# twosigma/Cook

Measured on AMD Instinct MI355X. Metric: match-cycles/sec at 1M pending x 50k offers, higher is better.
Workload: dtype f64

## Files before the change

### cook_amd/csrc/classfit_asm.hpp

```cpp
#pragma once
#if CF_SLOTS_N == 12
#define CF_O_CTRL "13728"
#define CF_O_CTRL4 "13732"
#define CF_O_ARR "15280"
#define CF_O_CLS32 "9504"
#define CF_SLOT_SHIFT "9"
#define CF_SLOT_N "12"
#elif CF_SLOTS_N == 24
#define CF_O_CTRL "16800"
#define CF_O_CTRL4 "16804"
#define CF_O_ARR "18352"
#define CF_O_CLS32 "12576"
#define CF_SLOT_SHIFT "10"
#define CF_SLOT_N "24"
#else
#error "CF_SLOTS_N: 12 or 24"
#endif
#ifndef CF_ASM_WAIT_READS
#define CF_ASM_WAIT_READS "30"
#endif
#define CF_ASM_MAX_STEP(ctrl) "v_max_f32_dpp v113, v113, v113 " ctrl "\n\ts_nop 1\n\t"
#define CF_ASM_DECIDER_STEP                                                                                                             \
  "v_readlane_b32 s60, v80, s44\n\t"                                                                                                    \
  "v_readlane_b32 s61, v81, s44\n\t"                                                                                                    \
  "v_readlane_b32 s62, v82, s44\n\t"                                                                                                    \
  "s_mov_b32 s41, 1\n\t"                                                                                                                \
  "s_and_b32 s63, s62, 0xffff00ff\n\t"                                                                                                   \
  "s_cmp_lg_u32 s63, 0\n\t"                                                                                                             \
  "s_cbranch_scc1 9f\n\t"                                                                                                               \
                                                                                           \
  "v_mov_b32_e32 v88, s47\n\t"                                                                                                          \
  "v_mov_b32_e32 v89, s51\n\t"                                                                                                          \
  "v_add_u32_e32 v100, s46, v83\n\t"                                                                                                    \
  "s_mov_b64 exec, 1\n\t"                                                                                                               \
  "ds_write_b32 v89, v88 offset:" CF_O_CTRL4 "\n\t"                                                                                              \
  "s_mov_b64 exec, -1\n\t"                                                                                                              \
  "s_mov_b32 s82, " CF_ASM_WAIT_READS "\n\t"              \
  "1:\n\t"                                                                                                                              \
  "ds_read_b32 v92, v100\n\t"                                                                                                           \
  "ds_read_b64 v[94:95], v100 offset:8\n\t"                                                                                             \
  "ds_read_b128 v[96:99], v100 offset:16\n\t"                                                                                           \
  "ds_read_b32 v93, v100\n\t"                                                                                                           \
  "v_lshlrev_b32_e32 v114, 3, v65\n\t"  \
  "v_add_u32_e32 v114, s56, v114\n\t"                                                                                                   \
  "ds_read_b64 v[114:115], v114\n\t"                                                                                                    \
                                        \
  "v_subrev_u32_e32 v101, s60, v71\n\t"                                                                                                 \
  "v_subrev_u32_e32 v102, s61, v72\n\t"                                                                                                 \
  "v_cvt_f64_u32_e32 v[104:105], v101\n\t"                                                                                              \
  "v_cvt_f64_u32_e32 v[106:107], v102\n\t"                                                                                              \
  "v_mul_f64 v[104:105], v[104:105], v[66:67]\n\t"                                                                                      \
  "v_mul_f64 v[106:107], v[106:107], v[68:69]\n\t"                                                                                      \
  "v_add_f64 v[104:105], v[104:105], v[106:107]\n\t"                                                                                    \
  "v_add_f64 v[104:105], -v[104:105], 1.0\n\t"                                                                                          \
  "v_cmp_le_u32_e64 s[64:65], s60, v71\n\t"                                                                                             \
  "v_cmp_le_u32_e64 s[66:67], s61, v72\n\t"                                                                                             \
  "v_cmp_ne_u32_e64 s[68:69], 0, v64\n\t"                                                                                               \
  "s_and_b64 s[64:65], s[64:65], s[66:67]\n\t"                                                                                          \
  "s_and_b64 s[64:65], s[64:65], s[68:69]\n\t"                                                                                          \
  "s_waitcnt lgkmcnt(0)\n\t"                                                                                                            \
        \
  "s_bfe_u32 s63, s62, 0x4000c\n\t"                                                                                                     \
  "s_cmp_eq_u32 s63, 0\n\t"                                                                                                             \
  "s_cbranch_scc1 3f\n\t"                                                                                                               \
  "v_readlane_b32 s66, v85, s44\n\t"                                                                                                    \
  "v_readlane_b32 s67, v86, s44\n\t"                                                                                                    \
  "s_cmp_lt_u32 s63, 1\n\t"                                                                                                           \
  "s_cbranch_scc1 3f\n\t"                                                                                                               \
  "s_bfe_u32 s72, s66, 0x100000\n\t"                                                                      \
  "s_lshr_b32 s73, s72, 8\n\t"                                                                                                          \
  "s_lshl_b32 s73, s73, 3\n\t"                                                                                                          \
  "s_and_b32 s72, s72, 0xff\n\t"                                                                                                        \
  "v_lshrrev_b64 v[108:109], s73, v[114:115]\n\t"                                                                                       \
  "v_and_b32_e32 v108, 0xff, v108\n\t"                                                                                                  \
  "v_cmp_eq_u32_e64 s[74:75], s72, v108\n\t"                                                                                            \
  "s_and_b64 s[64:65], s[64:65], s[74:75]\n\t"                                                                                          \
  "s_cmp_lt_u32 s63, 2\n\t"                                                                                                           \
  "s_cbranch_scc1 3f\n\t"                                                                                                               \
  "s_bfe_u32 s72, s66, 0x100010\n\t"                                                                      \
  "s_lshr_b32 s73, s72, 8\n\t"                                                                                                          \
  "s_lshl_b32 s73, s73, 3\n\t"                                                                                                          \
  "s_and_b32 s72, s72, 0xff\n\t"                                                                                                        \
  "v_lshrrev_b64 v[108:109], s73, v[114:115]\n\t"                                                                                       \
  "v_and_b32_e32 v108, 0xff, v108\n\t"                                                                                                  \
  "v_cmp_eq_u32_e64 s[74:75], s72, v108\n\t"                                                                                            \
  "s_and_b64 s[64:65], s[64:65], s[74:75]\n\t"                                                                                          \
  "s_cmp_lt_u32 s63, 3\n\t"                                                                                                           \
  "s_cbranch_scc1 3f\n\t"                                                                                                               \
  "s_bfe_u32 s72, s67, 0x100000\n\t"                                                                      \
  "s_lshr_b32 s73, s72, 8\n\t"                                                                                                          \
  "s_lshl_b32 s73, s73, 3\n\t"                                                                                                          \
  "s_and_b32 s72, s72, 0xff\n\t"                                                                                                        \
  "v_lshrrev_b64 v[108:109], s73, v[114:115]\n\t"                                                                                       \
// ... 23 lines not shown
  "v_cmp_ne_u32_e64 s[78:79], v109, v75\n\t"                                                                                            \
  "v_cmp_gt_i32_e64 s[80:81], 0, v95\n\t"                                                                                               \
  "s_and_b64 s[74:75], s[74:75], s[76:77]\n\t"                                                                                          \
  "s_and_b64 s[74:75], s[74:75], s[78:79]\n\t"                                                                                          \
  "s_or_b64 s[74:75], s[74:75], s[80:81]\n\t"                                                                                           \
  "s_and_b64 s[72:73], s[70:71], s[72:73]\n\t"                                          \
  "s_and_b64 s[70:71], s[72:73], s[74:75]\n\t"                                                                                            \
  "s_andn2_b64 s[76:77], s[52:53], s[70:71]\n\t"                                                                     \
  "s_cmp_eq_u64 s[76:77], 0\n\t"                                                                                                          \
  "s_cbranch_scc1 2f\n\t"                                                                                                                 \
   \
   \
  "s_and_b64 s[78:79], s[76:77], s[72:73]\n\t"                                                                                            \
  "s_cmp_eq_u64 s[78:79], 0\n\t"                                                                                                          \
  "s_cbranch_scc1 4f\n\t"                                                                                                                 \
  "v_and_b32_e32 v109, 0x3fff, v95\n\t"                                                                                                   \
  "s_and_b64 s[72:73], s[64:65], s[54:55]\n\t"                                                   \
  "10:\n\t"                                                                                                                               \
  "s_ff1_i32_b64 s83, s[78:79]\n\t"                                                                                                       \
  "v_readlane_b32 s63, v109, s83\n\t"                                                                                                     \
  "s_bitset0_b64 s[78:79], s83\n\t"                                                                                                       \
  "v_cmp_eq_u32_e64 vcc, s63, v65\n\t"                                                                                                    \
  "s_and_b64 vcc, vcc, s[72:73]\n\t"                                                                                                      \
  "s_cmp_eq_u64 vcc, 0\n\t"                                                                                                               \
  "s_cbranch_scc1 11f\n\t"                                                                                                                \
  "s_bitset1_b64 s[80:81], s83\n\t"                                                                                                       \
  "s_bitset0_b64 s[76:77], s83\n\t"                                                                                                       \
  "11:\n\t"                                                                                                                               \
  "s_cmp_lg_u64 s[78:79], 0\n\t"                                                                                                          \
  "s_cbranch_scc1 10b\n\t"                                                                                                                \
  "s_cmp_eq_u64 s[76:77], 0\n\t"                                                                                                          \
  "s_cbranch_scc1 2f\n\t"                                                                                                                 \
  "4:\n\t"                                                                                                                                \
  "s_sub_u32 s82, s82, 1\n\t"      \
  "s_cmp_eq_u32 s82, 0\n\t"                                                                                                             \
  "s_cbranch_scc1 9f\n\t"                                                                                                               \
  "s_sleep 1\n\t"                                                                                                                       \
  "s_branch 1b\n\t"                                                                                                                     \
  "2:\n\t"                                                                                                                              \
  "s_andn2_b64 s[74:75], s[52:53], s[80:81]\n\t"                                                                        \
  "s_or_b64 s[64:65], s[64:65], s[74:75]\n\t"                                                          \
  "v_cndmask_b32_e64 v110, v98, v104, s[54:55]\n\t"                                                                                     \
  "v_cndmask_b32_e64 v111, v99, v105, s[54:55]\n\t"                                                                                     \
  "v_cndmask_b32_e64 v110, 0, v110, s[64:65]\n\t"                                                                                       \
  "v_cndmask_b32_e64 v111, 0, v111, s[64:65]\n\t"                                                                                       \
  "v_cvt_f32_f64_e32 v112, v[110:111]\n\t"                                                                                              \
  "s_nop 0\n\t"                                                                                                                         \
  "v_mov_b32_e32 v113, v112\n\t"                                                                                                        \
  "s_nop 1\n\t"                                                                                                                         \
  CF_ASM_MAX_STEP("quad_perm:[1,0,3,2] row_mask:0xf bank_mask:0xf")                                                                     \
  CF_ASM_MAX_STEP("quad_perm:[2,3,0,1] row_mask:0xf bank_mask:0xf")                                                                     \
  CF_ASM_MAX_STEP("row_half_mirror row_mask:0xf bank_mask:0xf")                                                                         \
  CF_ASM_MAX_STEP("row_mirror row_mask:0xf bank_mask:0xf")                                                                              \
  CF_ASM_MAX_STEP("row_bcast:15 row_mask:0xa bank_mask:0xf")                                                                            \
  CF_ASM_MAX_STEP("row_bcast:31 row_mask:0xc bank_mask:0xf")                                                                            \
  "v_readlane_b32 s63, v113, 63\n\t"                                                                                                    \
  "s_mov_b32 s41, 0\n\t"                                                                                                                \
  "s_cmp_eq_u32 s63, 0\n\t"                                                                                                             \
  "s_cbranch_scc1 9f\n\t"                                                                                          \
  "s_mov_b32 s41, 1\n\t"                                                                                                                \
  "v_cmp_eq_f32_e64 s[78:79], s63, v112\n\t"                                                                                            \
  "v_add_f32_e32 v108, 0x35000000, v112\n\t"                                                                               \
  "v_cmp_le_f32_e64 s[76:77], s63, v108\n\t"                                                                                            \
  "v_and_b32_e32 v109, 0x40000000, v95\n\t"                                                                                             \
  "v_cmp_ne_u32_e64 s[70:71], 0, v109\n\t"                                                                                              \
  "s_and_b64 s[76:77], s[76:77], s[64:65]\n\t"                                      \
  "s_bcnt1_i32_b64 s62, s[76:77]\n\t"                                                                                                   \
  "s_cmp_gt_u32 s62, 1\n\t"                                                                                                             \
  "s_cbranch_scc1 9f\n\t"                                                                                                               \
  "s_and_b64 s[70:71], s[70:71], s[76:77]\n\t"                                                                                          \
  "s_and_b64 s[70:71], s[70:71], s[74:75]\n\t"                       \
  "s_cmp_lg_u64 s[70:71], 0\n\t"                                                                                                        \
  "s_cbranch_scc1 9f\n\t"                                                                                                               \
  "s_ff1_i32_b64 s82, s[78:79]\n\t"                                                                                                     \
  "s_cmp_lt_u32 s82, 58\n\t"                                                                                                            \
  "s_cbranch_scc0 5f\n\t"                                                                                                               \
                                                                                                         \
  "v_readlane_b32 s64, v71, s82\n\t"                                                                                                    \
  "v_readlane_b32 s65, v72, s82\n\t"                                                                                                    \
  "v_readlane_b32 s66, v65, s82\n\t"                                                                                                    \
  "s_sub_u32 s67, s64, s60\n\t"                                                                                                         \
  "s_sub_u32 s70, s65, s61\n\t"                                                                                                         \
  "v_cmp_eq_u32_e64 vcc, s82, v84\n\t"                                                                                                  \
  "v_mov_b32_e32 v88, s67\n\t"                                                                                                          \
  "v_mov_b32_e32 v89, s70\n\t"                                                                                                          \
  "s_cmp_lt_u32 s67, s49\n\t"                                                                                                           \
  "s_cselect_b32 s71, 1, 0\n\t"                                                                                                         \
  "s_cmp_lt_u32 s70, s50\n\t"                                                                                                           \
  "s_cselect_b32 s62, 1, 0\n\t"                                                                                                         \
  "s_or_b32 s71, s71, s62\n\t"                                                                                                          \
  "v_cndmask_b32_e32 v71, v71, v88, vcc\n\t"                                                                                            \
  "v_cndmask_b32_e32 v72, v72, v89, vcc\n\t"                                                                                            \
  "s_cmp_lg_u32 s71, 0\n\t"                                                                                                             \
  "s_cselect_b64 s[62:63], vcc, 0\n\t"                             \
  "s_mov_b32 s72, s44\n\t"                                                                                                              \
  "s_mov_b32 s73, 0\n\t"                                                                                                                \
  "v_cndmask_b32_e64 v64, v64, 0, s[62:63]\n\t"                                                                                         \
  "s_branch 7f\n\t"                                                                                                                     \
        \
  "5:\n\t"                                                                                                                              \
  "v_readlane_b32 s64, v96, s82\n\t"                                                                                                    \
  "v_readlane_b32 s65, v97, s82\n\t"                                                                                                    \
  "v_readlane_b32 s76, v95, s82\n\t"                                                                                                    \
  "v_readlane_b32 s77, v94, s82\n\t"                                                                                                    \
  "v_readlane_b32 s78, v73, s82\n\t"                                                                                                    \
  "s_sub_u32 s67, s64, s60\n\t"                                                                                                         \
// ... 33 lines not shown
  "s_nop 0\n\t"                                                                                                                         \
  "v_cndmask_b32_e32 v75, v75, v74, vcc\n\t"                                                                                            \
  "v_cndmask_b32_e32 v74, v74, v101, vcc\n\t"                                                                                           \
  "v_cndmask_b32_e32 v73, v73, v100, vcc\n\t"                                                                                           \
  "s_lshl_b32 s62, s80, 8\n\t"                                                                                                          \
  "s_lshl_b32 s63, s81, 12\n\t"                                                                                                         \
  "s_or_b32 s72, s44, s62\n\t"                                                                                                          \
  "s_or_b32 s72, s72, s63\n\t"                                                                                                          \
  "s_cmp_lg_u32 s71, 0\n\t"                                                                                                             \
  "s_cbranch_scc1 7f\n\t"                                                                              \
  "s_mul_i32 s62, s79, 56\n\t"                                                                                                          \
  "s_add_u32 s62, s62, s51\n\t"                                                                                                         \
  "v_mov_b32_e32 v90, s62\n\t"                                                                                                          \
  "ds_read_b128 v[116:119], v90 offset:" CF_O_CLS32 "\n\t"                                                                                        \
  "s_andn2_b64 s[62:63], s[54:55], s[68:69]\n\t"                                                                                        \
  "s_ff1_i32_b64 s83, s[62:63]\n\t"                                                                                                     \
  "v_cmp_eq_u32_e64 vcc, s83, v84\n\t"                                                                                                  \
  "v_mov_b32_e32 v88, s66\n\t"                                                                                                          \
  "v_mov_b32_e32 v89, s79\n\t"                                                                                                          \
  "v_mov_b32_e32 v91, s67\n\t"                                                                                                          \
  "v_mov_b32_e32 v101, s70\n\t"                                                                                                         \
  "v_cndmask_b32_e64 v64, v64, 1, vcc\n\t"                                                                                              \
  "v_cndmask_b32_e32 v65, v65, v88, vcc\n\t"                                                                                            \
  "v_cndmask_b32_e32 v70, v70, v89, vcc\n\t"                                                                                            \
  "v_cndmask_b32_e32 v71, v71, v91, vcc\n\t"                                                                                            \
  "v_cndmask_b32_e32 v72, v72, v101, vcc\n\t"                                                                                           \
  "s_waitcnt lgkmcnt(0)\n\t"                                                                                                            \
  "v_cndmask_b32_e32 v66, v66, v116, vcc\n\t"                                                                                           \
  "v_cndmask_b32_e32 v67, v67, v117, vcc\n\t"                                                                                           \
  "v_cndmask_b32_e32 v68, v68, v118, vcc\n\t"                                                                                           \
  "v_cndmask_b32_e32 v69, v69, v119, vcc\n\t"                                                                                           \
   \
  "7:\n\t"                                                                                                                              \
  "v_cmp_eq_u32_e64 vcc, s44, v84\n\t"                                                                                                  \
  "v_mov_b32_e32 v88, s66\n\t"                                                                                                          \
  "v_cmp_lt_u32_e64 s[62:63], s67, v80\n\t"                                                                                             \
  "v_cmp_lt_u32_e64 s[76:77], s70, v81\n\t"                                                                                             \
  "v_cndmask_b32_e32 v76, v76, v88, vcc\n\t"                                                                                            \
  "s_or_b64 s[62:63], s[62:63], s[76:77]\n\t"                                                                                           \
  "s_lshl_b64 s[76:77], -2, s44\n\t"                                                                                                    \
  "s_and_b64 s[62:63], s[62:63], s[76:77]\n\t"                                                                                          \
  "s_or_b64 s[38:39], s[38:39], s[62:63]\n\t"                                                                                           \
  "s_min_u32 s37, s37, s67\n\t"                                                                                                         \
  "s_min_u32 s40, s40, s70\n\t"                                                                                                         \
  "s_add_u32 s36, s36, 1\n\t"                                                                                                           \
  "v_mov_b32_e32 v88, s72\n\t"                                                                                                          \
  "v_mov_b32_e32 v89, s73\n\t"                                                                                                          \
  "v_mov_b32_e32 v90, s64\n\t"                                                                                                          \
  "v_mov_b32_e32 v91, s65\n\t"                                                                                                          \
  "v_mov_b32_e32 v100, s48\n\t"                                                                                                         \
  "s_mov_b64 exec, 1\n\t"                                                                                                               \
  "ds_write_b128 v100, v[88:91]\n\t"                                                                                                    \
  "s_mov_b64 exec, -1\n\t"                                                                                                              \
  "s_mov_b32 s41, 2\n\t"                                                                                                                \
  "9:\n\t"

#define CF_ASM_CLASS_STEP                                                                                                               \
  "v_mov_b32_e32 v80, s44\n\t"                                                                                                          \
  "s_lshl_b32 s60, s45, 2\n\t"                                                                                                          \
  "s_add_u32 s60, s60, s44\n\t"                                                                                                         \
  "v_mov_b32_e32 v81, s60\n\t"                                                                                                          \
  "ds_read_b64 v[82:83], v80 offset:" CF_O_CTRL "\n\t"                                                                     \
  "ds_read_b32 v84, v81 offset:" CF_O_CTRL4 "\n\t"                                                                   \
  "s_mov_b32 s41, 3\n\t"                                                                                                                \
  "s_waitcnt lgkmcnt(0)\n\t"                                                                                                            \
  "v_readfirstlane_b32 s61, v82\n\t"                                                                                                    \
  "v_readfirstlane_b32 s42, v83\n\t"                                                                                                    \
  "v_readfirstlane_b32 s43, v84\n\t"                                                                                                    \
  "s_cmp_lg_u32 s61, 0\n\t"                                                                                                             \
  "s_cbranch_scc1 9f\n\t"                                                                                                               \
  "s_cmp_lg_u32 s43, s40\n\t"                                                                                                           \
  "s_cbranch_scc1 9f\n\t"                                                                                                               \
  "s_mov_b32 s41, 2\n\t"                                                                                                                \
                                                                                                 \
  "1:\n\t"                                                                                                                              \
  "s_cmp_eq_u64 s[36:37], 0\n\t"                                                                                                        \
  "s_cbranch_scc1 9f\n\t"                                                                                                               \
  "s_cmp_eq_u32 s39, s56\n\t"                                                                                                           \
  "s_cbranch_scc1 2f\n\t"                                                                                                               \
  "s_add_u32 s62, s36, -1\n\t"                                                                                                          \
  "s_addc_u32 s63, s37, -1\n\t"                                                                                                         \
  "s_and_b64 s[36:37], s[36:37], s[62:63]\n\t"                                                                                          \
  "s_add_u32 s38, s38, 1\n\t"                                                                                                           \
  "s_add_u32 s39, s39, 1\n\t"                                                                                                           \
  "s_cmp_eq_u32 s39, s57\n\t"                                                                                                           \
  "s_cselect_b32 s39, 0, s39\n\t"                                                                                                       \
  "s_branch 1b\n\t"                                                                                                                     \
  "2:\n\t"                                                                                                                                \
// ... 123 lines not shown
```

### cook_amd/csrc/classfit_walk.hpp

```cpp
#pragma once
#if defined(CF_PROF) && !defined(CF_STATS)
#define CF_STATS 1
#endif
#ifdef CF_STATS
#define CF_STAT(x) x
#define CF_TICKS() cook_ticks()
#else
#define CF_STAT(x) ((void)0)
#define CF_TICKS() 0ull
#endif
#ifdef CF_PROF
#define CF_PROF_T(x) const unsigned long long x = __builtin_readcyclecounter()
#define CF_PROF_ADD(i, d) prof[i] += (unsigned long long)(d)
#else
#define CF_PROF_T(x) ((void)0)
#define CF_PROF_ADD(i, d) ((void)0)
#endif

#ifndef CF_AHEAD
#define CF_AHEAD 10
#endif
constexpr unsigned CF_BOARD = CF_AHEAD;
#ifndef CF_SLOTS_N
#define CF_SLOTS_N 12
// ... 285 lines not shown
  v.id = (unsigned)wave_read_lane((int)p.w0, (int)wl), v.pos = (unsigned)wave_read_lane((int)p.pos, (int)wl), v.fc = (unsigned)wave_read_lane((int)p.fc, (int)wl),
  v.fm = (unsigned)wave_read_lane((int)p.fm, (int)wl), v.cls = (unsigned)wave_read_lane((int)p.cls, (int)wl), v.aux = (unsigned)wave_read_lane((int)p.aux, (int)wl);
  return v;
}
static __device__ __forceinline__ unsigned cf_poll(const uint32_t* p) { return (unsigned)wave_read_lane((int)ld_wg(p), 0); }
static __device__ __forceinline__ unsigned long long cf_below(unsigned s) { return (1ull << s) - 1ull; }

enum : unsigned { CFE_K = 0, CFE_M, CFE_NP, CFE_NCLS, CFE_NKIND, CFE_CMIN, CFE_MMIN, CFE_KC, CFE_KM, CFE_MINFC, CFE_MINFM, CFE_N = 12 };
constexpr float CF_BAND32 = 1.0f / 2097152.0f;

struct CfFixed {
  CfEnt board[CF_SLOTS * 8u];
  CfLog log[64];
  CfJob ring[2u * 64u];
  CfPost post2[8];
  CfClass cls[CF_MAXCLS];
  uint32_t pw[8u * CF_LV], aw[8u * CF_LV], gk[CF_MAXKIND * CF_LV], ovt[CF_LV];
  uint32_t ctrl[8];
  uint32_t ovl[192], ckept[3u * CF_MAXCLS], misc[CFX_N];
  uint32_t env_t[CF_LV], envw[CFE_N];
};
static_assert(sizeof(CfFixed) % 16 == 0, "the arrays behind it are 16-byte aligned");
#if COOK_HAS_ASM_WALK
#define CF_ASM_EPOCH_LIVE "57"
#include "classfit_asm.hpp"
static_assert(CF_EPOCH_AT == 58 && CF_OVL == 58, "classfit_asm.hpp: the overlay's size");
static_assert(offsetof(CfFixed, ctrl) == 13728 + (CF_SLOTS - 12) * 256 && offsetof(CfFixed, cls) == 9472 + (CF_SLOTS - 12) * 256 && sizeof(CfFixed) == 15280 + (CF_SLOTS - 12) * 256 && sizeof(CfClass) == 56 && offsetof(CfClass, hTc) == 32 &&
                  offsetof(CfClass, hTm) == 40 && offsetof(CfEnt, pos) == 8 && offsetof(CfEnt, cid) == 12 && offsetof(CfEnt, fc) == 16 && offsetof(CfEnt, fa) == 24 && sizeof(CfEnt) == 32 &&
                  sizeof(CfLog) == 32 && offsetof(CfLog, ofc) == 8,
              "classfit_asm.hpp: offsets of the LDS records");
typedef unsigned cf_u32x16 __attribute__((ext_vector_type(16)));
typedef unsigned cf_u32x8 __attribute__((ext_vector_type(8)));
typedef unsigned cf_u32x4 __attribute__((ext_vector_type(4)));
#endif

template <int ROLE>
static __device__ __forceinline__ void cf_walk_role(const CfLds& S, const MatchState& st, const CfBuf& b, const unsigned lw, const unsigned rep, const unsigned nrep,
                                                    const unsigned long long t_start) {
  constexpr bool is_decider = ROLE == 0, is_class_wave = ROLE == 1, is_books = ROLE == 2;
  const unsigned tid = threadIdx.x, lane = lane_id();
  CfCtl* ctl = b.ctl;
  const unsigned K = wave_uniform_u32(S.envw[CFE_K]), cmin = wave_uniform_u32(S.envw[CFE_CMIN]), mmin = wave_uniform_u32(S.envw[CFE_MMIN]);
  const uint32_t* t = S.t;
#define n_cls wave_uniform_u32(S.envw[CFE_NCLS])
#define n_kind wave_uniform_u32(S.envw[CFE_NKIND])
#define NP wave_uniform_u32(S.envw[CFE_NP])
  CfChunkLane c;
  unsigned nch_wave = 0;
  cf_setup_chunks(S.cls, n_cls, is_class_wave ? lw : 0xFFu, lane, c, nch_wave);
  c.lv = CfLv8{0u, 0u, 0u, 0u, 0u, 0u, 0u, 0u}, c.la = c.lv;
  unsigned my_kinds = 0;
  {
    const unsigned forw = is_class_wave ? lw : (is_decider && lane >= CF_OVL ? lane - CF_OVL + 1u : 0xFFu);
    for (unsigned ci = 0; ci < n_cls; ++ci)
      if (S.cls[ci].wave == forw && S.cls[ci].kind < 32u) my_kinds |= 1u << S.cls[ci].kind;
  }
  const unsigned wk = is_class_wave ? wave_uniform_u32(my_kinds) : 0u;
  unsigned one_cls = 0xFFFFFFFFu, u_off = 0, u_n = 0;
  double u_hTc = 0.0, u_hTm = 0.0;
  auto class_setup = [&] {
    unsigned cnt = 0, ci0 = 0;
    for (unsigned ci = 0; ci < n_cls; ++ci)
      if (S.cls[ci].wave == lw) ++cnt, ci0 = ci;
    one_cls = cnt == 1u ? ci0 : 0xFFFFFFFFu;
    const CfClass* cl = &S.cls[ci0];
    u_off = cl->off, u_n = cl->n, u_hTc = cl->hTc, u_hTm = cl->hTm;
  };
  if (is_class_wave) {
    class_setup();
    for (unsigned ch = 0; ch < nch_wave; ++ch) cf_tighten(S, lane, ch, c);
    if (rep == 0u && lw != 0u) cf_wave_tables(S, lw, lane, c, wk, n_kind);
  }
  CfOvLane o;
  o.valid = 0u, o.id = 0u, o.cls = 0u, o.fc = 0u, o.fm = 0u, o.hTc = 0.0, o.hTm = 0.0;
  unsigned nrm = 0, rm1 = 0xFFFFFFFFu, rm2 = 0xFFFFFFFFu;
  unsigned minfc_all = wave_uniform_u32(S.envw[CFE_MINFC]), minfm_all = wave_uniform_u32(S.envw[CFE_MINFM]);
  unsigned matched = 0, head = 0;
  unsigned jc = 0, jm = 0, jmeta = 0, jgrp = 0, jeq0 = 0, jeq1 = 0, jnov0 = 0, jnov1 = 0;
  int res = -1;
  unsigned long long b1m = 0ull;
  unsigned seen = 0, gen = 0;
  unsigned tight_applied = 0;
  bool bk_room0 = false, nx_room0 = false, nx_walk = false;
  unsigned st_scans = 0, st_exact = 0, st_open = 0, st_ovwin = 0, st_gpu = 0, st_epochs = 0, st_tight = 0, st_walked = 0, st_dead = 0, st_opendead = 0, st_spins = 0, st_flips = 0,
           st_rewinds = 0;
  unsigned long long tk_epoch = 0, tk_books = 0, tk_walk = 0, tk_phase1 = 0;
#ifdef CF_PROF
  unsigned long long prof[8] = {0, 0, 0, 0, 0, 0, 0, 0};
#endif
  auto job_of = [&](unsigned s) -> CfJobU {
    CfJobU J;
    J.c = (unsigned)wave_read_lane((int)jc, (int)s), J.m = (unsigned)wave_read_lane((int)jm, (int)s);
    const unsigned meta = (unsigned)wave_read_lane((int)jmeta, (int)s);
    J.kind = meta & 255u, J.L = (meta >> 8) & 15u, J.n_eq = (meta >> 12) & 15u, J.n_nov = (meta >> 16) & 15u, J.grouped = (meta >> 20) & 1u;
    J.grp = 0u, J.eq0 = J.eq1 = 0u, J.nov0 = J.nov1 = 0xFFFFFFFFu;
    if (meta >> 12) {
      J.grp = (unsigned)wave_read_lane((int)jgrp, (int)s), J.eq0 = (unsigned)wave_read_lane((int)jeq0, (int)s), J.eq1 = (unsigned)wave_read_lane((int)jeq1, (int)s),
      J.nov0 = (unsigned)wave_read_lane((int)jnov0, (int)s), J.nov1 = (unsigned)wave_read_lane((int)jnov1, (int)s);
    }
    return J;
  };
  auto tables_room_any = [&](unsigned L, unsigned m) -> bool {
    bool r = S.ovt[L] > m;
    for (unsigned x = 1; x <= (unsigned)CF_CW; ++x) r = r || S.aw[x * CF_LV + L] > m;
    return r;
  };
  auto tables_walk = [&](unsigned kind, unsigned L, unsigned m) -> bool {
    bool r = false;
    if (kind == 0u) {
      r = S.ovt[L] > m;
      for (unsigned x = 1; x <= (unsigned)CF_CW; ++x) r = r || S.pw[x * CF_LV + L] > m;
    } else if (kind < (unsigned)CF_MAXKIND) {
      r = S.gk[kind * CF_LV + L] > m;
    }
    return r;
  };
  CfJob nxt;
  nxt.c = nxt.m = nxt.meta = nxt.grp = nxt.eq[0] = nxt.eq[1] = nxt.nov[0] = nxt.nov[1] = 0u;
  auto books_next = [&](unsigned nbase) {
    const unsigned nn = nbase < K ? cf_min(64u, K - nbase) : 0u;
    const unsigned nslot = (nbase >> 6) & 1u;
// ... 38 lines not shown
    unsigned cur_ord = 0;
    unsigned ph = 0;
    bool batch_done = nw == 0u;
    const unsigned long long tw0 = CF_TICKS();
    CF_PROF_T(cw0);
    while (!batch_done) {
      unsigned md = 0;
      if (is_decider) {
#if COOK_HAS_ASM_WALK
        cf_u32x16 ST = {0u, 0u, 0u, 0u, 0u, 0u, 0u, 0u, 0u, 0u, 0u, 0u, 0u, 0u, 0u, 0u};
        cf_u32x8 JB = {jc, jm, jmeta, clw * 32u, lane, jeq0, jeq1, 0u};
        const unsigned long long rel0 = cook_ballot(!isov & ((my_kinds & 1u) != 0u)), ovm = cf_below(CF_OVL);
        const cf_u32x8 MK = {wave_uniform_u32((unsigned)rel0), wave_uniform_u32((unsigned)(rel0 >> 32)), wave_uniform_u32((unsigned)ovm), wave_uniform_u32((unsigned)(ovm >> 32)),
                             wave_uniform_u32(cook_lds_off(S.attr8)), 0u, 0u, 0u};
        const unsigned a_board = wave_uniform_u32(cook_lds_off(S.board)), a_log = wave_uniform_u32(cook_lds_off(S.log));
        auto st_pack = [&] {
          const unsigned long long hc = (unsigned long long)__double_as_longlong(o.hTc), hm = (unsigned long long)__double_as_longlong(o.hTm);
          ST[0] = o.valid, ST[1] = o.id, ST[2] = (unsigned)hc, ST[3] = (unsigned)(hc >> 32), ST[4] = (unsigned)hm, ST[5] = (unsigned)(hm >> 32), ST[6] = o.cls, ST[7] = o.fc, ST[8] = o.fm,
          ST[9] = nrm, ST[10] = rm1, ST[11] = rm2, ST[12] = (unsigned)res;
        };
        auto st_unpack = [&] {
          o.valid = ST[0], o.id = ST[1], o.hTc = __longlong_as_double((long long)((unsigned long long)ST[3] << 32 | ST[2])),
          o.hTm = __longlong_as_double((long long)((unsigned long long)ST[5] << 32 | ST[4])), o.cls = ST[6], o.fc = ST[7], o.fm = ST[8], nrm = ST[9], rm1 = ST[10], rm2 = ST[11],
          res = (int)ST[12];
        };
#endif
        while (md == 0u) {
          todo = wave_uniform_u64(todo), cur_ord = wave_uniform_u32(cur_ord), logn = wave_uniform_u32(logn), matched = wave_uniform_u32(matched), gen = wave_uniform_u32(gen);
          minfc_all = wave_uniform_u32(minfc_all), minfm_all = wave_uniform_u32(minfm_all), b1m = wave_uniform_u64(b1m);
#if COOK_HAS_ASM_WALK
          {
            st_pack();
            CF_PROF_T(f0);
            while (todo != 0ull) {
              const unsigned fs = (unsigned)__ffsll(todo) - 1u;
#define CF_U(x) wave_uniform_u32((unsigned)(x))
              cf_u32x8 SC = {CF_U(matched), CF_U(minfc_all), CF_U(b1m), CF_U(b1m >> 32), CF_U(minfm_all), 1u, 0u, 0u};
              const cf_u32x8 AR = {CF_U(fs), CF_U((base + fs) << 12 | (gen & 15u) << 8), CF_U(a_board + cf_slot(cur_ord) * 8u * (unsigned)sizeof(CfEnt)), CF_U(fs | cur_ord << 8),
                                   CF_U(a_log + logn * (unsigned)sizeof(CfLog)), CF_U(cmin), CF_U(mmin), a_board};
#undef CF_U
              asm volatile(CF_ASM_DECIDER_STEP
                           : "+{v[64:79]}"(ST), "+{s[36:43]}"(SC)
                           : "{v[80:87]}"(JB), "{s[44:51]}"(AR), "{s[52:59]}"(MK)
                           : "v88", "v89", "v90", "v91", "v92", "v93", "v94", "v95", "v96", "v97", "v98", "v99", "v100", "v101", "v102", "v103", "v104", "v105", "v106", "v107", "v108",
                             "v109", "v110", "v111", "v112", "v113", "v114", "v115", "v116", "v117", "v118", "v119", "s60", "s61", "s62", "s63", "s64", "s65", "s66", "s67", "s68", "s69",
                             "s70", "s71", "s72", "s73", "s74", "s75", "s76", "s77", "s78", "s79", "s80", "s81", "s82", "s83", "vcc", "scc", "memory");
#ifdef CF_DELAY_D
              __builtin_amdgcn_s_sleep(6);
#endif
              const unsigned status = wave_uniform_u32(SC[5]);
              if (status == 1u) break;
              matched = wave_uniform_u32(SC[0]), minfc_all = wave_uniform_u32(SC[1]), minfm_all = wave_uniform_u32(SC[4]);
              b1m = wave_uniform_u64((unsigned long long)SC[3] << 32 | SC[2]);
              logn += status >> 1;
              todo &= todo - 1ull, ++cur_ord;
              CF_PROF_ADD(4, 1);
            }
            CF_PROF_T(f1);
            CF_PROF_ADD(5, f1 - f0);
            WAIT_LDS();
            st_unpack();
          }
#endif
          if (todo == 0ull) {
            md = CFM_BATCH_END;
            st_lane0_b32(&S.ctrl[0], md);
            break;
          }
          CF_PROF_T(p0);
          const unsigned s = (unsigned)__ffsll(todo) - 1u;
          const unsigned ord = cur_ord;
          st_lane0_b32(&S.ctrl[1], s | ord << 8);
          const unsigned Jc = (unsigned)wave_read_lane((int)jc, (int)s), Jm = (unsigned)wave_read_lane((int)jm, (int)s), meta = (unsigned)wave_read_lane((int)jmeta, (int)s);
          const unsigned kind = meta & 255u;
          const unsigned want = (base + s) << 12 | (gen & 15u) << 8;
          const CfEnt* e = &S.board[cf_slot(ord) * 8u + clw];
          const bool relevant = !isov && kind < 32u && ((my_kinds >> (kind & 31u)) & 1u);
          unsigned cpos, ccid, cfc, cfm;
          double cfa;
          bool acc;
          bool ok_ov = isov & (o.valid != 0u) & (kind == 0u) & (o.fc >= Jc) & (o.fm >= Jm);
          if (meta >> 12) {
            const CfJobU J = job_of(s);
            ok_ov = ok_ov & cf_cons_ok(S, J, o.id, ok_ov);
          }
          for (;;) {
            const unsigned t1 = ld_wg(&e->tag);
            COMPILER_FENCE();
            cpos = e->pos, ccid = e->cid, cfc = e->fc, cfm = e->fm, cfa = e->fa;
// ... 550 lines not shown
        if (unm) {
          fail = (((bb >> lane) & 1ull) ? 1u : 0u) | (room ? 2u : 0u);
          if (fail == 0u) fail = 8u;
        }
        st.fail_code[base + lane] = fail;
      }
      books_next(base + 64u);
      bk_room0 = nx_room0;
      if (base + 128u + lane < K) nxt = b.jobs[base + 128u + lane];
      tk_books += CF_TICKS() - tb0;
    }
    EMU_SITE("classfit: batch end");
    __syncthreads();
  }
  if (is_decider) {
    if (lane == 0) {
      st.summary[0] = matched;
      st.summary[1] = (matched == 0u || head) ? 1u : 0u;
      st.summary[2] = st_epochs;
      const unsigned long long t_end = cook_ticks();
      uint32_t* sx = ctl->stats;
      sx[CFS_MATCHED] = matched, sx[CFS_OV_WIN] = st_ovwin, sx[CFS_OPEN] = st_open, sx[CFS_OPEN_DEAD] = st_opendead, sx[CFS_GPU_PLACE] = st_gpu, sx[CFS_EPOCHS] = st_epochs,
      sx[CFS_EXACT] = st_exact, sx[CFS_WALKED] = st_walked, sx[CFS_DEAD_DROP] = st_dead, sx[CFS_BATCHES] = (K + 63u) / 64u, sx[CFS_PRESETTLED] = K - st_walked;
      sx[CFS_TICKS_TOTAL] = (uint32_t)(t_end - t_start), sx[CFS_TICKS_PROLOGUE] = (uint32_t)(t_loop - t_start), sx[CFS_TICKS_EPOCH] = (uint32_t)tk_epoch;
      sx[CFS_TICKS_WALK] = (uint32_t)tk_walk, sx[CFS_TICKS_PHASE1] = (uint32_t)tk_phase1;
      sx[CFS_HWID_DECIDER] = cook_hw_id();
    }
    const unsigned sp = wave_max_u32(!isov ? st_spins : 0u);
    if (lane == 0) ctl->stats[CFS_SPINS] = sp;
  }
  if (is_class_wave && lane == 0) atomicAdd(&ctl->stats[CFS_SCANS], st_scans), atomicAdd(&ctl->stats[CFS_TIGHTEN], st_tight), atomicAdd(&ctl->stats[CFS_REWINDS], st_rewinds);
  if (is_books && lane == 0) ctl->stats[CFS_TICKS_PRECHECK] = (uint32_t)tk_books, ctl->stats[CFS_FLIPS] = st_flips, ctl->stats[CFS_HWID_BOOKS] = cook_hw_id();
#ifdef CF_PROF
  if (lane == 0 && (is_decider || (is_class_wave && lw >= 1u && lw <= 2u && rep == 0u)))
    for (int i = 0; i < 8; ++i) ctl->stats[24 + 8 * (is_decider ? 0u : lw) + i] = (uint32_t)(prof[i] >> 4);
#endif
#undef n_cls
#undef n_kind
#undef NP
}

static __device__ __forceinline__ void cf_walk_pool(char* lds, const MatchIn* __restrict__ inp, const MatchState& st, const CfBuf& b) {
  const unsigned tid = threadIdx.x, lane = lane_id(), w = wave_id();
  CfCtl* ctl = b.ctl;
  const unsigned K = inp->K, M = ctl->M, G = inp->G;
  const unsigned NP = (M + 63u) & ~63u;
  const unsigned long long t_start = cook_ticks();
  const bool any_eq = ctl->any_eq != 0u, any_group = ctl->any_group != 0u;
  __shared__ unsigned s_total, s_wsum[CF_WAVES];
  constexpr unsigned GPT = CF_MAXG / CF_THREADS;
  unsigned gsz[GPT];
  unsigned gsum = 0;
#pragma unroll
  for (unsigned x = 0; x < GPT; ++x) {
    const unsigned g = tid * GPT + x;
    unsigned sz = 0;
    if (any_group && g < G && b.gcount[g] != 0u) sz = (inp->g_run_off ? inp->g_run_off[g + 1] - inp->g_run_off[g] : 0u) + b.gcount[g];
    gsz[x] = sz, gsum += sz;
  }
  unsigned incl = gsum;
  for (unsigned d = 1; d < 64u; d <<= 1) {
    const unsigned y = shfl_up_t<unsigned>(incl, d);
    if (lane >= d) incl += y;
  }
  if (lane == 63u) s_wsum[w] = incl;
  __syncthreads();
  unsigned wbase = 0;
  for (unsigned x = 0; x < w; ++x) wbase += s_wsum[x];
// ... 115 lines not shown
```

### cook_amd/csrc/engine.hip

```cpp
#include <hip/hip_runtime.h>
#include <sys/mman.h>
#include <ucontext.h>

#include <algorithm>
#include <atomic>
#include <cmath>
#include <cstdlib>
#include <chrono>
#include <cstring>
#include <limits>
#include <functional>
#include <map>
#include <string>
#include <tuple>
#include <vector>

#include "../../include/cookmatch.h"
#include "common.hpp"
#include "multi.hpp"
#include "considerable_kernels.hpp"
#include "match_kernels.hpp"
#include "match_v2.hpp"
#include "classfit.hpp"
#include "offers_kernels.hpp"
// ... 1297 lines not shown
  return true;
}
void cf_run(cook_engine* lead, cook_engine* const* es, unsigned n, hipStream_t stream) {
  cook_engine* e = lead;
  for (unsigned i0 = 0; i0 < n; i0 += (unsigned)CF_PACK) {
    const unsigned c = std::min<unsigned>(CF_PACK, n - i0);
    CfPack pk{};
    for (unsigned x = 0; x < (unsigned)CF_PACK; ++x) pk.c[x] = es[i0 + (x < c ? x : 0u)]->deferred_cf;
    KLS("cf_walk", stream, cf_walk, c, CF_THREADS, pk);
  }
  for (unsigned i = 0; i < n; ++i) {
    const CfPoolCtx& c = es[i]->deferred_cf;
    const unsigned G = es[i]->last_in.G;
    if (G) KLS("cf_group_chains", stream, cf_group_chains, div_up(G, 256), 256, c.b, c.st, G);
  }
  constexpr size_t SLOT = 16 + 48 * 4;
  if (!lead->h_cf) COOK_HIP(hipHostMalloc((void**)&lead->h_cf, 64 * SLOT, hipHostMallocDefault));
  if (n > 64) lead->fail(COOK_E_INVALID, "cook_cycle_match_multi: at most 64 pools per call");
  for (unsigned i = 0; i < n; ++i) {
    char* slot = lead->h_cf + i * SLOT;
    COOK_HIP(hipMemcpyAsync(slot, es[i]->deferred_cf.st.summary, 16, hipMemcpyDeviceToHost, stream));
    COOK_HIP(hipMemcpyAsync(slot + 16, es[i]->deferred_cf.b.ctl->stats, 48 * 4, hipMemcpyDeviceToHost, stream));
  }
  COOK_HIP(hipStreamSynchronize(stream));
  for (unsigned i = 0; i < n; ++i) {
    cook_engine* x = es[i];
    const unsigned* sum = (const unsigned*)(lead->h_cf + i * SLOT);
    if (sum[3] == 0xDEADu) lead->fail(COOK_E_STATE, "cf_walk: the pool's tables do not fit the workgroup's LDS (the host's check let it through)");
    std::memcpy(x->cf_stats, lead->h_cf + i * SLOT + 16, 48 * 4);
#ifdef CF_PROF
    {
      const uint32_t* q = x->cf_stats;
      std::fprintf(stderr, "CFPROF (x16 shader cycles) decider: slow steps %u (candidates %u evaluation %u commit %u) plain steps %u in %u walk-total %u | class wave 1: poll %u answer %u answers %u idle %u idles %u | class wave 2: poll %u answer %u answers %u idle %u idles %u | walk ticks(100MHz) %u\n", q[27], q[24], q[25], q[26], q[28], q[29], q[31], q[32], q[33], q[35], q[36], q[37], q[40], q[41], q[43], q[44], q[45], q[CFS_TICKS_WALK]);
    }
#endif
    WinCtl c{};
    c.matched = sum[0], c.head_matched = sum[1], c.rounds = sum[2], c.head = x->last_in.K, c.visited_sum = x->cf_stats[CFS_WALKED];
    c.t_seq = x->cf_stats[CFS_TICKS_TOTAL], c.t_setup = x->cf_stats[CFS_TICKS_PROLOGUE];
    x->last_ctl = c;
    x->last_form = 3;
    x->has_deferred_cf = false;
    x->has_deferred = false;
    x->match_done = true;
  }
}

void match_run_device(cook_engine* e, unsigned K, const uint32_t* j_index, bool defer = false) {
  MatchIn in = e->min;
  in.K = K;
  in.j_index = j_index;
  in.good_enough = e->params.good_enough_fitness;
  in.host_lifetime_mins = e->params.host_lifetime_mins;
  const unsigned M = in.M, G = in.G;
  e->last_in = in;
  e->last_in_valid = true;
  MatchState st;
  st.ac = e->m_ac.ensure(M);
  st.am = e->m_am.ensure(M);
  st.acount = e->m_acount.ensure(M);
  st.group_last = e->m_group_last.ensure(G);
  st.job_prev = e->m_job_prev.ensure(K);
  st.job_to_offer = e->m_j2o.ensure(K);
  st.fail_code = e->m_fail.ensure(K);
  st.summary = e->m_summary.ensure(4);
  st.alive = e->m_alive.ensure((M + 63u) / 64u + 1u);
  st.jmin = (const double*)e->m_jmin.ensure(4);
// ... 1295 lines not shown
```

Before: 21.15.

## Run decider loop inside inline asm and prefetch next slot's row during commit

The decider's per-step loop moves from C++ into the assembly block, so one asm call walks every bit in the todo mask and the per-step register marshalling and exit checks go away. During each step's commit path it issues the LDS reads for the next slot's row early, so the next step can skip those reads and only post its head word. The loads are waited on with partial lgkmcnt counts instead of a full drain. This adds complexity and relies on careful lgkmcnt accounting, and opt-in profiling hooks for the individual phases are added as well.

```diff
diff --git a/cook_amd/csrc/classfit_asm.hpp b/cook_amd/csrc/classfit_asm.hpp
--- a/cook_amd/csrc/classfit_asm.hpp
+++ b/cook_amd/csrc/classfit_asm.hpp
@@ -19,8 +19,57 @@
 #ifndef CF_ASM_WAIT_READS
 #define CF_ASM_WAIT_READS "30"
 #endif
+#define CF_ASM_READ_ROW(addr)                                                                                                           \
+  "ds_read_b32 v92, " addr "\n\t"                                                                                                       \
+  "ds_read_b64 v[94:95], " addr " offset:8\n\t"                                                                                         \
+  "ds_read_b128 v[96:99], " addr " offset:16\n\t"                                                                                       \
+  "ds_read_b32 v93, " addr "\n\t"                                                                                                       \
+  "v_lshlrev_b32_e32 v114, 3, v65\n\t"                                                                                                  \
+  "v_add_u32_e32 v114, s56, v114\n\t"                                                                                                   \
+  "ds_read_b64 v[114:115], v114\n\t"
+#define CF_ASM_HEAD_WORD "s_mov_b64 exec, 1\n\tds_write_b32 v89, v88 offset:" CF_O_CTRL4 "\n\ts_mov_b64 exec, -1\n\t"
+#ifdef CF_PROF_PHASES
+#define CF_ASM_WAIT_COLD "s_waitcnt lgkmcnt(0)\n\t"
+#define CF_ASM_WAIT_EARLY "s_waitcnt lgkmcnt(0)\n\t"
+#else
+#define CF_ASM_WAIT_COLD "s_waitcnt lgkmcnt(1)\n\t"
+#define CF_ASM_WAIT_EARLY "s_waitcnt lgkmcnt(2)\n\t"
+#endif
 #define CF_ASM_MAX_STEP(ctrl) "v_max_f32_dpp v113, v113, v113 " ctrl "\n\ts_nop 1\n\t"
-#define CF_ASM_DECIDER_STEP                                                                                                             \
+#ifdef CF_DELAY_D
+#define CF_ASM_DELAY_D "s_sleep 6\n\t"
+#else
+#define CF_ASM_DELAY_D ""
+#endif
+#ifdef CF_PROF_PHASES
+#define CF_ASM_PS(acc) "s_memtime s[84:85]\n\ts_waitcnt lgkmcnt(0)\n\ts_sub_u32 s86, s84, s87\n\ts_add_u32 " acc ", " acc ", s86\n\ts_mov_b32 s87, s84\n\t"
+#define CF_ASM_PS_ENTRY "s_memtime s[84:85]\n\ts_waitcnt lgkmcnt(0)\n\ts_mov_b32 s87, s84\n\t"
+#define CF_ASM_PS_TOP "s_memtime s[84:85]\n\t"
+#define CF_ASM_PS_READ "s_sub_u32 s86, s84, s87\n\ts_add_u32 s92, s92, s86\n\ts_mov_b32 s87, s84\n\t" CF_ASM_PS("s88")
+#define CF_ASM_PS_REREAD "s_add_u32 s93, s93, 1\n\t"
+#else
+#define CF_ASM_PS(acc) ""
+#define CF_ASM_PS_ENTRY ""
+#define CF_ASM_PS_TOP ""
+#define CF_ASM_PS_READ ""
+#define CF_ASM_PS_REREAD ""
+#endif
+#define CF_ASM_DECIDER_RUN                                                                                                              \
+  CF_ASM_PS_ENTRY                                                                                                                       \
+                     \
+  "0:\n\t"                                                                                                                              \
+  CF_ASM_PS_TOP                                                                                                                         \
+  "s_ff1_i32_b64 s44, s[42:43]\n\t"                                                                                                    \
+  "s_lshl_b32 s45, s44, 12\n\t"                                                                                                        \
+  "s_or_b32 s45, s45, s58\n\t"                                                                                                         \
+  "s_lshl_b32 s47, s57, 8\n\t"                                                                                                         \
+  "s_or_b32 s47, s47, s44\n\t"                                                                                                         \
+  "s_mul_i32 s46, s57, 43\n\t"                                                           \
+  "s_lshr_b32 s46, s46, " CF_SLOT_SHIFT "\n\t"                                                                                          \
+  "s_mul_i32 s46, s46, " CF_SLOT_N "\n\t"                                                                                               \
+  "s_sub_u32 s46, s57, s46\n\t"                                                                                                        \
+  "s_lshl_b32 s46, s46, 8\n\t"                                                                                                         \
+  "s_add_u32 s46, s46, s51\n\t"                                                                                                        \
   "v_readlane_b32 s60, v80, s44\n\t"                                                                                                    \
   "v_readlane_b32 s61, v81, s44\n\t"                                                                                                    \
   "v_readlane_b32 s62, v82, s44\n\t"                                                                                                    \
@@ -28,22 +77,26 @@
   "s_and_b32 s63, s62, 0xffff00ff\n\t"                                                                                                   \
   "s_cmp_lg_u32 s63, 0\n\t"                                                                                                             \
   "s_cbranch_scc1 9f\n\t"                                                                                                               \
-                                                                                           \
+   \
+   \
+  "v_add_u32_e32 v100, s46, v83\n\t"                                                                                                    \
   "v_mov_b32_e32 v88, s47\n\t"                                                                                                          \
   "v_mov_b32_e32 v89, s51\n\t"                                                                                                          \
-  "v_add_u32_e32 v100, s46, v83\n\t"                                                                                                    \
-  "s_mov_b64 exec, 1\n\t"                                                                                                               \
-  "ds_write_b32 v89, v88 offset:" CF_O_CTRL4 "\n\t"                                                                                              \
-  "s_mov_b64 exec, -1\n\t"                                                                                                              \
   "s_mov_b32 s82, " CF_ASM_WAIT_READS "\n\t"              \
-  "1:\n\t"                                                                                                                              \
-  "ds_read_b32 v92, v100\n\t"                                                                                                           \
-  "ds_read_b64 v[94:95], v100 offset:8\n\t"                                                                                             \
-  "ds_read_b128 v[96:99], v100 offset:16\n\t"                                                                                           \
-  "ds_read_b32 v93, v100\n\t"                                                                                                           \
-  "v_lshlrev_b32_e32 v114, 3, v65\n\t"  \
-  "v_add_u32_e32 v114, s56, v114\n\t"                                                                                                   \
-  "ds_read_b64 v[114:115], v114\n\t"                                                                                                    \
+  "s_cmp_lg_u32 s59, 0\n\t"                                                                                                              \
+  "s_mov_b32 s59, 0\n\t"                                                                                                                 \
+  "s_cbranch_scc1 13f\n\t"                             \
+  CF_ASM_READ_ROW("v100")                                                                                                               \
+  CF_ASM_HEAD_WORD                                                                                                                      \
+  CF_ASM_WAIT_COLD                                                                                                                      \
+  "s_branch 15f\n\t"                                                                                                                    \
+  "13:\n\t"                                                                                                                             \
+  CF_ASM_HEAD_WORD                                                                                                                      \
+  "s_branch 15f\n\t"                                                                                                                    \
+  "1:\n\t"                                                                                                               \
+  CF_ASM_READ_ROW("v100")                                                                                                               \
+  "s_waitcnt lgkmcnt(0)\n\t"                                                                                                            \
+  "15:\n\t"                                                                                                                             \
                                         \
   "v_subrev_u32_e32 v101, s60, v71\n\t"                                                                                                 \
   "v_subrev_u32_e32 v102, s61, v72\n\t"                                                                                                 \
@@ -58,7 +111,8 @@
   "v_cmp_ne_u32_e64 s[68:69], 0, v64\n\t"                                                                                               \
   "s_and_b64 s[64:65], s[64:65], s[66:67]\n\t"                                                                                          \
   "s_and_b64 s[64:65], s[64:65], s[68:69]\n\t"                                                                                          \
-  "s_waitcnt lgkmcnt(0)\n\t"                                                                                                            \
+  CF_ASM_WAIT_EARLY                                                                                                                     \
+  CF_ASM_PS_READ                                                                                                                        \
         \
   "s_bfe_u32 s63, s62, 0x4000c\n\t"                                                                                                     \
   "s_cmp_eq_u32 s63, 0\n\t"                                                                                                             \
@@ -148,12 +202,14 @@
   "s_cmp_eq_u64 s[76:77], 0\n\t"                                                                                                          \
   "s_cbranch_scc1 2f\n\t"                                                                                                                 \
   "4:\n\t"                                                                                                                                \
+  CF_ASM_PS_REREAD                                                                                                                      \
   "s_sub_u32 s82, s82, 1\n\t"      \
   "s_cmp_eq_u32 s82, 0\n\t"                                                                                                             \
   "s_cbranch_scc1 9f\n\t"                                                                                                               \
   "s_sleep 1\n\t"                                                                                                                       \
   "s_branch 1b\n\t"                                                                                                                     \
   "2:\n\t"                                                                                                                              \
+  CF_ASM_PS("s89")                                                                                                                      \
   "s_andn2_b64 s[74:75], s[52:53], s[80:81]\n\t"                                                                        \
   "s_or_b64 s[64:65], s[64:65], s[74:75]\n\t"                                                          \
   "v_cndmask_b32_e64 v110, v98, v104, s[54:55]\n\t"                                                                                     \
@@ -188,6 +244,7 @@
   "s_and_b64 s[70:71], s[70:71], s[74:75]\n\t"                       \
   "s_cmp_lg_u64 s[70:71], 0\n\t"                                                                                                        \
   "s_cbranch_scc1 9f\n\t"                                                                                                               \
+  CF_ASM_PS("s90")                                                                                                                      \
   "s_ff1_i32_b64 s82, s[78:79]\n\t"                                                                                                     \
   "s_cmp_lt_u32 s82, 58\n\t"                                                                                                            \
   "s_cbranch_scc0 5f\n\t"                                                                                                               \
@@ -287,6 +344,22 @@
   "v_cndmask_b32_e32 v69, v69, v119, vcc\n\t"                                                                                           \
    \
   "7:\n\t"                                                                                                                              \
+   \
+  "s_add_u32 s74, s42, -1\n\t"                                                                                                          \
+  "s_addc_u32 s75, s43, -1\n\t"                                                                                                         \
+  "s_and_b64 s[74:75], s[74:75], s[42:43]\n\t"                                                                                          \
+  "s_cbranch_scc0 14f\n\t"                                                                             \
+  "s_add_u32 s83, s57, 1\n\t"                                                                                                           \
+  "s_mul_i32 s78, s83, 43\n\t"                                                                                                          \
+  "s_lshr_b32 s78, s78, " CF_SLOT_SHIFT "\n\t"                                                                                          \
+  "s_mul_i32 s78, s78, " CF_SLOT_N "\n\t"                                                                                               \
+  "s_sub_u32 s83, s83, s78\n\t"                                                                                                         \
+  "s_lshl_b32 s83, s83, 8\n\t"                                                                                                          \
+  "s_add_u32 s83, s83, s51\n\t"                                                                                                         \
+  "v_add_u32_e32 v103, s83, v83\n\t"                                                                                                    \
+  "s_mov_b32 s59, 1\n\t"                                                                                                                \
+  CF_ASM_READ_ROW("v103")                                                                                                               \
+  "14:\n\t"                                                                                                                             \
   "v_cmp_eq_u32_e64 vcc, s44, v84\n\t"                                                                                                  \
   "v_mov_b32_e32 v88, s66\n\t"                                                                                                          \
   "v_cmp_lt_u32_e64 s[62:63], s67, v80\n\t"                                                                                             \
@@ -308,7 +381,22 @@
   "ds_write_b128 v100, v[88:91]\n\t"                                                                                                    \
   "s_mov_b64 exec, -1\n\t"                                                                                                              \
   "s_mov_b32 s41, 2\n\t"                                                                                                                \
-  "9:\n\t"
+  "9:\n\t"                                                                                                                              \
+  CF_ASM_PS("s91")                                                                                                                      \
+                      \
+  "s_cmp_eq_u32 s41, 1\n\t"                                                                                                             \
+  "s_cbranch_scc1 8f\n\t"                                                                                                               \
+  CF_ASM_DELAY_D                                                                                                                        \
+  "s_lshr_b32 s60, s41, 1\n\t"                                                                                                          \
+  "s_lshl_b32 s60, s60, 5\n\t"                                                                                                          \
+  "s_add_u32 s48, s48, s60\n\t"                                                                  \
+  "s_add_u32 s57, s57, 1\n\t"                                                                                                           \
+  "s_add_u32 s60, s42, -1\n\t"                                                                                                          \
+  "s_addc_u32 s61, s43, -1\n\t"                                                                                                         \
+  "s_and_b64 s[42:43], s[42:43], s[60:61]\n\t"                                                                                          \
+  "s_cbranch_scc1 0b\n\t"                                                                                                               \
+  "8:\n\t"                                                                                                                              \
+  "s_waitcnt lgkmcnt(0)\n\t"
 
 #define CF_ASM_CLASS_STEP                                                                                                               \
   "v_mov_b32_e32 v80, s44\n\t"                                                                                                          \
diff --git a/cook_amd/csrc/classfit_walk.hpp b/cook_amd/csrc/classfit_walk.hpp
--- a/cook_amd/csrc/classfit_walk.hpp
+++ b/cook_amd/csrc/classfit_walk.hpp
@@ -341,6 +341,12 @@
 typedef unsigned cf_u32x16 __attribute__((ext_vector_type(16)));
 typedef unsigned cf_u32x8 __attribute__((ext_vector_type(8)));
 typedef unsigned cf_u32x4 __attribute__((ext_vector_type(4)));
+typedef unsigned cf_u32x2 __attribute__((ext_vector_type(2)));
+#ifdef CF_PROF_PHASES
+#define CF_PS_OPS , "+{s[84:91]}"(PS), "+{s[92:93]}"(PS2)
+#else
+#define CF_PS_OPS
+#endif
 #endif
 
 template <int ROLE>
@@ -396,6 +402,9 @@
   unsigned long long tk_epoch = 0, tk_books = 0, tk_walk = 0, tk_phase1 = 0;
 #ifdef CF_PROF
   unsigned long long prof[8] = {0, 0, 0, 0, 0, 0, 0, 0};
+#endif
+#ifdef CF_PROF_PHASES
+  unsigned long long prof2[8] = {0, 0, 0, 0, 0, 0, 0, 0};
 #endif
   auto job_of = [&](unsigned s) -> CfJobU {
     CfJobU J;
@@ -500,29 +509,34 @@
           {
             st_pack();
             CF_PROF_T(f0);
-            while (todo != 0ull) {
-              const unsigned fs = (unsigned)__ffsll(todo) - 1u;
+            if (todo != 0ull) {
 #define CF_U(x) wave_uniform_u32((unsigned)(x))
-              cf_u32x8 SC = {CF_U(matched), CF_U(minfc_all), CF_U(b1m), CF_U(b1m >> 32), CF_U(minfm_all), 1u, 0u, 0u};
-              const cf_u32x8 AR = {CF_U(fs), CF_U((base + fs) << 12 | (gen & 15u) << 8), CF_U(a_board + cf_slot(cur_ord) * 8u * (unsigned)sizeof(CfEnt)), CF_U(fs | cur_ord << 8),
-                                   CF_U(a_log + logn * (unsigned)sizeof(CfLog)), CF_U(cmin), CF_U(mmin), a_board};
+              cf_u32x8 SC = {CF_U(matched), CF_U(minfc_all), CF_U(b1m), CF_U(b1m >> 32), CF_U(minfm_all), 1u, CF_U(todo), CF_U(todo >> 32)};
+              cf_u32x8 AR = {0u, 0u, 0u, 0u, CF_U(a_log + logn * (unsigned)sizeof(CfLog)), CF_U(cmin), CF_U(mmin), a_board};
+              cf_u32x8 MR = MK;
+              MR[5] = CF_U(cur_ord), MR[6] = CF_U(base << 12 | (gen & 15u) << 8), MR[7] = 0u;
 #undef CF_U
-              asm volatile(CF_ASM_DECIDER_STEP
-                           : "+{v[64:79]}"(ST), "+{s[36:43]}"(SC)
-                           : "{v[80:87]}"(JB), "{s[44:51]}"(AR), "{s[52:59]}"(MK)
+#ifdef CF_PROF_PHASES
+              cf_u32x8 PS = {0u, 0u, 0u, 0u, 0u, 0u, 0u, 0u};
+              cf_u32x2 PS2 = {0u, 0u};
+#endif
+              asm volatile(CF_ASM_DECIDER_RUN
+                           : "+{v[64:79]}"(ST), "+{s[36:43]}"(SC), "+{s[44:51]}"(AR), "+{s[52:59]}"(MR) CF_PS_OPS
+                           : "{v[80:87]}"(JB)
                            : "v88", "v89", "v90", "v91", "v92", "v93", "v94", "v95", "v96", "v97", "v98", "v99", "v100", "v101", "v102", "v103", "v104", "v105", "v106", "v107", "v108",
                              "v109", "v110", "v111", "v112", "v113", "v114", "v115", "v116", "v117", "v118", "v119", "s60", "s61", "s62", "s63", "s64", "s65", "s66", "s67", "s68", "s69",
                              "s70", "s71", "s72", "s73", "s74", "s75", "s76", "s77", "s78", "s79", "s80", "s81", "s82", "s83", "vcc", "scc", "memory");
-#ifdef CF_DELAY_D
-              __builtin_amdgcn_s_sleep(6);
-#endif
-              const unsigned status = wave_uniform_u32(SC[5]);
-              if (status == 1u) break;
               matched = wave_uniform_u32(SC[0]), minfc_all = wave_uniform_u32(SC[1]), minfm_all = wave_uniform_u32(SC[4]);
               b1m = wave_uniform_u64((unsigned long long)SC[3] << 32 | SC[2]);
-              logn += status >> 1;
-              todo &= todo - 1ull, ++cur_ord;
-              CF_PROF_ADD(4, 1);
+              todo = wave_uniform_u64((unsigned long long)SC[7] << 32 | SC[6]);
+              const unsigned ord1 = wave_uniform_u32(MR[5]);
+              CF_PROF_ADD(4, ord1 - cur_ord);
+#ifdef CF_PROF_PHASES
+              for (int i = 0; i < 4; ++i) prof2[i] += wave_uniform_u32(PS[4 + i]);
+              prof2[4] += wave_uniform_u32(PS2[0]), prof2[5] += wave_uniform_u32(PS2[1]), prof2[6] += 1u;
+#endif
+              cur_ord = ord1;
+              logn = wave_uniform_u32((AR[4] - a_log) / (unsigned)sizeof(CfLog));
             }
             CF_PROF_T(f1);
             CF_PROF_ADD(5, f1 - f0);
@@ -1139,8 +1153,17 @@
   if (is_class_wave && lane == 0) atomicAdd(&ctl->stats[CFS_SCANS], st_scans), atomicAdd(&ctl->stats[CFS_TIGHTEN], st_tight), atomicAdd(&ctl->stats[CFS_REWINDS], st_rewinds);
   if (is_books && lane == 0) ctl->stats[CFS_TICKS_PRECHECK] = (uint32_t)tk_books, ctl->stats[CFS_FLIPS] = st_flips, ctl->stats[CFS_HWID_BOOKS] = cook_hw_id();
 #ifdef CF_PROF
-  if (lane == 0 && (is_decider || (is_class_wave && lw >= 1u && lw <= 2u && rep == 0u)))
+#ifdef CF_PROF_PHASES
+  constexpr unsigned cf_prof_waves = 1u;
+#else
+  constexpr unsigned cf_prof_waves = 2u;
+#endif
+  if (lane == 0 && (is_decider || (is_class_wave && lw >= 1u && lw <= cf_prof_waves && rep == 0u)))
     for (int i = 0; i < 8; ++i) ctl->stats[24 + 8 * (is_decider ? 0u : lw) + i] = (uint32_t)(prof[i] >> 4);
+#endif
+#ifdef CF_PROF_PHASES
+  if (is_decider && lane == 0)
+    for (int i = 0; i < 8; ++i) ctl->stats[40 + i] = (uint32_t)(i < 5 ? prof2[i] >> 4 : prof2[i]);
 #endif
 #undef n_cls
 #undef n_kind
diff --git a/cook_amd/csrc/engine.hip b/cook_amd/csrc/engine.hip
--- a/cook_amd/csrc/engine.hip
+++ b/cook_amd/csrc/engine.hip
@@ -1353,6 +1353,10 @@
     {
       const uint32_t* q = x->cf_stats;
       std::fprintf(stderr, "CFPROF (x16 shader cycles) decider: slow steps %u (candidates %u evaluation %u commit %u) plain steps %u in %u walk-total %u | class wave 1: poll %u answer %u answers %u idle %u idles %u | class wave 2: poll %u answer %u answers %u idle %u idles %u | walk ticks(100MHz) %u\n", q[27], q[24], q[25], q[26], q[28], q[29], q[31], q[32], q[33], q[35], q[36], q[37], q[40], q[41], q[43], q[44], q[45], q[CFS_TICKS_WALK]);
+#ifdef CF_PROF_PHASES
+      std::fprintf(stderr, "CFPHASES (x16 shader cycles) plain step: rows landed %u answers accepted %u decision %u commit+books %u tail %u | re-reads %u runs %u\n", q[40], q[41], q[42], q[43],
+                   q[44], q[45], q[46]);
+#endif
     }
 #endif
     WinCtl c{};
```

New measurement: 21.06 (median of 2 runs). About the same (-0.4%).
